# Chatit-cloud/BEE2BEE

Measured on AMD Instinct MI355X. Metric: output tokens/sec (llama3-8b bf16 greedy decode, replica peers), higher is better.
Workload: dtype bf16; 1 GPU; model=llama3-8b, global_batch=1536, seq_len=1024, parallelism=replica-dp1, decode_graphs=True, distinct_prompts=256

## Files before the change

bee2bee_amd/engine/runner.py:

```python
from __future__ import annotations

from typing import List, Optional, Tuple

import torch
import torch.nn.functional as F

from .. import ops
from ..models.spec import ModelSpec
from ..models.weights import ModelWeights
from .kv import PagedKV


class Runner:
    def __init__(
        self,
        spec: ModelSpec,
        weights: ModelWeights,
        kv: PagedKV,
        device: torch.device,
        dtype: torch.dtype = torch.bfloat16,
        layer_range: Optional[Tuple[int, int]] = None,
        window: Optional[int] = None,
    ) -> None:
        self.spec = spec
        self.weights = weights
        self.kv = kv
        self.device = device
        self.dtype = dtype
        self.layer_lo, self.layer_hi = layer_range or (0, spec.n_layers)
        self.scale = spec.head_dim**-0.5
        self.window = int(
            (spec.sliding_window or 0) if window is None else window)
        self.ep = None
        self.tp_group = None
        self.decode_attn_fn = None
        self.kv_observer = None
        cos, sin = ops.rope_tables(
            spec.max_seq_len, spec.head_dim, spec.rope_theta, device,
            scaling=spec.rope_scaling,
        )
        self.rope_cos, self.rope_sin = cos, sin

    @property
    def is_first_stage(self) -> bool:
        return self.layer_lo == 0

    @property
    def is_last_stage(self) -> bool:
        return self.layer_hi == self.spec.n_layers


    def embed(self, input_ids: torch.Tensor,
              positions: Optional[torch.Tensor] = None) -> torch.Tensor:
        h = F.embedding(input_ids, self.weights.embed)
        if self.spec.pos_type == "learned" and positions is not None:
            h = h + F.embedding(positions.long(), self.weights.pos_embed)
        return h

    def _norm(self, x, w, b):
        if self.spec.norm_type == "layernorm":
            return ops.layernorm(x, w, b, self.spec.rms_eps)
        return ops.rmsnorm(x, w, self.spec.rms_eps)

    def _fused_add_norm(self, x, resid, w, b):
        if self.spec.norm_type == "layernorm":
            return ops.fused_add_layernorm(x, resid, w, b, self.spec.rms_eps)
        return ops.fused_add_rmsnorm(x, resid, w, self.spec.rms_eps)

    def lm_head(self, hidden: torch.Tensor) -> torch.Tensor:
        normed = self._norm(hidden, self.weights.final_norm,
                            self.weights.final_norm_bias)
        return F.linear(normed, self.weights.lm_head)

    def _layer(
        self,
        layer_idx: int,
        hidden: torch.Tensor,
        residual: Optional[torch.Tensor],
        positions: torch.Tensor,
        slot_mapping: torch.Tensor,
        attn_fn,
    ) -> Tuple[torch.Tensor, torch.Tensor]:
        s = self.spec
        lw = self.weights.layers[layer_idx]
        if residual is None:
            residual = hidden
            normed = self._norm(hidden, lw.attn_norm, lw.attn_norm_bias)
        else:
            normed, residual = self._fused_add_norm(
                hidden, residual, lw.attn_norm, lw.attn_norm_bias
            )

        qkv = F.linear(normed, lw.wqkv)
        if lw.wqkv_bias is not None:
            qkv = qkv + lw.wqkv_bias
        T = qkv.shape[0]
        q, k, v = qkv.split([s.q_size, s.kv_size, s.kv_size], dim=-1)
        q = q.view(T, s.n_heads, s.head_dim)
        k = k.view(T, s.n_kv_heads, s.head_dim)
        v = v.view(T, s.n_kv_heads, s.head_dim)
        if s.qk_norm:
            ops.qk_norm_rope_inplace(q, k, positions, self.rope_cos,
                                     self.rope_sin, lw.q_norm, lw.k_norm,
                                     s.rms_eps)
        elif s.pos_type == "rope":
            ops.rope_inplace(q, k, positions, self.rope_cos, self.rope_sin)
        if self.kv_observer is not None:
            self.kv_observer(layer_idx, k, v)
        k_cache, v_cache = self.kv.layer(layer_idx)
        sc = self.kv.layer_scales(layer_idx)
        if sc is None:
            ops.kv_cache_store(k, v, k_cache, v_cache, slot_mapping)
        else:
            ops.kv_cache_store(k, v, k_cache, v_cache, slot_mapping,
                               k_inv_scale=sc[2], v_inv_scale=sc[3])
        attn_out = attn_fn(layer_idx, q, k, v, k_cache, v_cache)
        attn_out = F.linear(attn_out.reshape(T, s.q_size), lw.wo, lw.wo_bias)
        if self.tp_group is not None:
            import torch.distributed as dist

            dist.all_reduce(attn_out, group=self.tp_group)

        normed, residual = self._fused_add_norm(
            attn_out, residual, lw.mlp_norm, lw.mlp_norm_bias
        )
        if s.is_moe:
            mlp_out = self._moe_mlp(lw, normed)
        elif s.act_type == "gelu":
            fc = F.linear(normed, lw.w_gate_up, lw.w_gate_up_bias)
            mlp_out = F.linear(ops.gelu(fc), lw.w_down, lw.w_down_bias)
        else:
            gate_up = F.linear(normed, lw.w_gate_up)
            mlp_out = F.linear(ops.swiglu(gate_up), lw.w_down)
            if self.tp_group is not None:
                import torch.distributed as dist

                dist.all_reduce(mlp_out, group=self.tp_group)
        return mlp_out, residual

# ... 83 lines not shown
            out.index_add_(
                0, tok, contrib * weights.reshape(-1).unsqueeze(-1)
            )
            return out.to(x.dtype)

        out = torch.zeros_like(x, dtype=torch.float32)
        for e in range(E):
            mask = idx == e
            if not bool(mask.any()):
                continue
            tok, kslot = mask.nonzero(as_tuple=True)
            xe = x[tok]
            ge = F.linear(xe, lw.moe_w_gate_up[e])
            ye = F.linear(ops.swiglu(ge), lw.moe_w_down[e])
            out.index_add_(0, tok, ye.float() * weights[tok, kslot, None])
        return out.to(x.dtype)

    def _run_layers(
        self,
        hidden: torch.Tensor,
        positions: torch.Tensor,
        slot_mapping: torch.Tensor,
        attn_fn,
    ) -> torch.Tensor:
        residual = None
        for layer_idx in range(self.layer_lo, self.layer_hi):
            hidden, residual = self._layer(
                layer_idx, hidden, residual, positions, slot_mapping, attn_fn
            )
        return hidden + residual if residual is not None else hidden

    def forward_prefill(
        self,
        input_ids_or_hidden: torch.Tensor,
        positions: torch.Tensor,
        slot_mapping: torch.Tensor,
        cu_seqlens: torch.Tensor,
        max_seqlen: int,
        block_table: Optional[torch.Tensor] = None,
        seq_lens: Optional[torch.Tensor] = None,
        query_lens: Optional[torch.Tensor] = None,
    ) -> torch.Tensor:
        chunked = seq_lens is not None

        def attn(layer_idx, q, k, v, k_cache, v_cache):
            if chunked:
                sc = self.kv.layer_scales(layer_idx)
                kw = {} if sc is None else {"k_scale": sc[0],
                                            "v_scale": sc[1]}
                if self.window:
                    kw["window"] = self.window
# ... 25 lines not shown
        def attn(layer_idx, q, k, v, k_cache, v_cache):
            sc = self.kv.layer_scales(layer_idx)
            kw = {} if sc is None else {"k_scale": sc[0], "v_scale": sc[1]}
            if self.decode_attn_fn is not None:
                if self.window:
                    raise ValueError(
                        "sliding-window attention is not supported with an "
                        "injected (context-parallel) decode attention")
                return self.decode_attn_fn(
                    q, k_cache, v_cache, block_table, seq_lens, self.scale,
                    **kw
                )
            if self.window:
                kw["window"] = self.window
            return ops.attn_decode(
                q, k_cache, v_cache, block_table, seq_lens, self.scale, **kw
            )

        hidden = (
            self.embed(input_ids_or_hidden, positions)
            if self.is_first_stage
            else input_ids_or_hidden
        )
        return self._run_layers(hidden, positions, slot_mapping, attn)
```

bee2bee_amd/ops/__init__.py:

```python
from __future__ import annotations

import os
from typing import Optional, Tuple

import torch

from . import reference

_hip = None
_hip_err: Optional[str] = None


def _load_hip():
    global _hip, _hip_err
    if _hip is not None or _hip_err is not None:
        return _hip
    try:
        import importlib

        _hip = importlib.import_module("bee2bee_amd.ops._bee2bee_hip")
    except Exception as e:
        _hip_err = str(e)
        _hip = None
    return _hip
# ... 139 lines not shown
    q: torch.Tensor,
    k_cache: torch.Tensor,
    v_cache: torch.Tensor,
    block_table: torch.Tensor,
    seq_lens: torch.Tensor,
    scale: float,
    k_scale: Optional[torch.Tensor] = None,
    v_scale: Optional[torch.Tensor] = None,
    window: int = 0,
    path="auto",
    max_z: int = 0,
):
    if _use_hip(q):
        out, ml = require_hip().attn_decode_select(
            q, k_cache, v_cache, block_table, seq_lens, scale, k_scale,
            v_scale, window, _DECODE_PATHS.get(path, path), max_z
        )
        return out, ml
    return reference.attn_decode_lse(
        q, k_cache, v_cache, block_table, seq_lens, scale,
        k_scale=k_scale, v_scale=v_scale, window=window)


def attn_prefill(
    q: torch.Tensor,
    k: torch.Tensor,
    v: torch.Tensor,
    cu_seqlens: torch.Tensor,
    max_seqlen: int,
    scale: float,
    causal: bool = True,
    window: int = 0,
) -> torch.Tensor:
    if _use_hip(q):
        return require_hip().attn_prefill(
            q, k, v, cu_seqlens, max_seqlen, scale, causal, window
        )
    return reference.attn_prefill(q, k, v, cu_seqlens, max_seqlen, scale,
                                  causal, window=window)


def attn_prefill_paged(
    q: torch.Tensor,
    k_cache: torch.Tensor,
    v_cache: torch.Tensor,
    block_table: torch.Tensor,
# ... 57 lines not shown
```

bee2bee_amd/ops/csrc/attn_decode.hip:

```cpp
#include "common.h"

#define DEC_BLOCK 256
#define DEC_WAVES 4
#define DEC_CHUNK 256

template <typename KVT>
__device__ __forceinline__ bf16x8 load_kv_bf16x8(const KVT* p);
template <>
__device__ __forceinline__ bf16x8 load_kv_bf16x8(const unsigned short* p) {
    return *reinterpret_cast<const bf16x8*>(p);
}
template <>
__device__ __forceinline__ bf16x8 load_kv_bf16x8(const unsigned char* p) {
    float f[8];
    load_fp8x8(p, f);
    bf16x8 r;
#pragma unroll
    for (int e = 0; e < 8; ++e) r[e] = (__bf16)f[e];
    return r;
}
template <typename KVT> struct kv_pair_t;
template <> struct kv_pair_t<unsigned short> { short2v v; };
template <> struct kv_pair_t<unsigned char> { u8x2 v; };
__device__ __forceinline__ float2v kv_pair_f32(kv_pair_t<unsigned short> p) {
// ... 710 lines not shown
    for (int c = c0; c < nc; ++c) Ltot += __expf(ml_s[c][0] - M) * ml_s[c][1];
    const float inv = (Ltot > 0.f) ? 1.f / Ltot : 0.f;
    if (out_ml != nullptr && threadIdx.x == 0) {
        float* mlrow = out_ml + ((long)b * nq + kvh * G + g) * 2;
        mlrow[0] = M;
        mlrow[1] = Ltot;
    }

    for (int d = threadIdx.x; d < hd; d += DEC_BLOCK) {
        float acc = 0.f;
        for (int c = c0; c < nc; ++c)
            acc += __expf(ml_s[c][0] - M) *
                   part_o[((base + c) * G + g) * hd + d];
        out[((long)b * nq + kvh * G + g) * hd + d] = f2bf(acc * inv);
    }
}

__device__ __forceinline__ int phase_tid() {
    int t = threadIdx.x;
    asm volatile("" : "+v"(t));
    return t;
}

template <int G, int HD, bool FOLD, typename KVT, bool SCALED, bool WINDOWED>
__global__ __launch_bounds__(DEC_BLOCK)
__attribute__((amdgpu_waves_per_eu(4))) void attn_decode_fused_kernel(
    const unsigned short* __restrict__ q,
    const KVT* __restrict__ k_cache,
    const KVT* __restrict__ v_cache,
    const int* __restrict__ block_table,
    const int* __restrict__ seq_lens,
    float* __restrict__ part_o,
    float* __restrict__ part_ml,
    unsigned short* __restrict__ out,
    float* __restrict__ out_ml,
    int nkv, int W, int bs, int C, long q_stride, float scale,
    const float* __restrict__ k_scale,
    const float* __restrict__ v_scale,
    int window) {
    constexpr int KSTEPS = HD / 32;
    constexpr int TILES = WAVE / 16;
    const int b = blockIdx.x;
    const int kvh = blockIdx.y;
    const int nq = nkv * G;
    const int L = seq_lens[b];
    const int lo = WINDOWED ? max(0, L - window) : 0;
    const int c0 = WINDOWED ? lo / DEC_CHUNK : 0;
    if ((c0 + (int)blockIdx.z) * DEC_CHUNK >= L) {
        if (FOLD && L <= 0) {
            unsigned short* orow = out + ((long)b * nq + kvh * G) * HD;
            for (int i = threadIdx.x; i < G * HD; i += DEC_BLOCK) orow[i] = 0;
            if (out_ml != nullptr && threadIdx.x < G) {
                float* mlrow =
                    out_ml + ((long)b * nq + kvh * G + threadIdx.x) * 2;
                mlrow[0] = -1e30f;
                mlrow[1] = 0.f;
            }
        }
        return;
    }
    float ksc = 1.f, vsc = 1.f;
    if (SCALED) {
        ksc = k_scale[kvh];
        vsc = v_scale[kvh];
    }
    extern __shared__ __attribute__((aligned(16))) char smem_raw[];
    float* p_s = reinterpret_cast<float*>(smem_raw);
    long* voff_s = reinterpret_cast<long*>(p_s + DEC_CHUNK * G);
    float* merge = reinterpret_cast<float*>(voff_s + DEC_CHUNK);
    float* run = merge + DEC_WAVES * G * HD;
    unsigned short* q_s = reinterpret_cast<unsigned short*>(run + G * HD);
    float* red = reinterpret_cast<float*>(
        reinterpret_cast<char*>(q_s) + ((G * HD * 2 + 15) & ~15));
    float* runml = red + DEC_WAVES * G * 2;

    {
    const int lane = threadIdx.x % WAVE;
    const int wid = threadIdx.x / WAVE;
    if (SCALED) {
        float amax = 0.f;
        for (int i = threadIdx.x; i < G * HD; i += DEC_BLOCK) {
            const int g = i / HD, d = i % HD;
            amax = fmaxf(amax, fabsf(bf2f(f2bf(
                bf2f(q[(long)b * q_stride + (kvh * G + g) * (long)HD + d]) *
                scale))));
        }
        amax = wave_max(amax);
        if (lane == 0) red[wid] = amax;
        __syncthreads();
        amax = fmaxf(fmaxf(red[0], red[1]), fmaxf(red[2], red[3]));
        const int e = __builtin_amdgcn_readfirstlane(
            (__float_as_int(amax) >> 23) & 0xff);
        float qmul = 1.f;
        if (e >= 8 && e < 122) {
            qmul = __int_as_float((261 - e) << 23);
            ksc *= __int_as_float((e - 7) << 23);
        }
        for (int i = threadIdx.x; i < G * HD; i += DEC_BLOCK) {
            const int g = i / HD, d = i % HD;
            q_s[i] = f2bf(bf2f(f2bf(
                bf2f(q[(long)b * q_stride + (kvh * G + g) * (long)HD + d]) *
                scale)) * qmul);
// ... 258 lines not shown

template <int G, int HD, typename KVT, bool WIN>
static void launch_scores_mfma(
    dim3 grid, int smem, hipStream_t stream, const unsigned short* q,
    const KVT* kc, const int* block_table, const int* seq_lens,
    unsigned short* p_buf, float* part_ml, int nkv, int W, int bs, int C,
    long q_stride, float scale, const float* k_scale, int window) {
    if constexpr (sizeof(KVT) == 1) {
        if (k_scale != nullptr) {
            hipLaunchKernelGGL(
                (attn_scores_mfma_kernel<G, HD, KVT, true, WIN>), grid,
                dim3(DEC_BLOCK), smem, stream, q, kc, block_table, seq_lens,
                p_buf, part_ml, nkv, W, bs, C, q_stride, scale, k_scale,
                window);
            return;
        }
    }
    hipLaunchKernelGGL((attn_scores_mfma_kernel<G, HD, KVT, false, WIN>),
                       grid, dim3(DEC_BLOCK), smem, stream, q, kc,
                       block_table, seq_lens, p_buf, part_ml, nkv, W, bs, C,
                       q_stride, scale, nullptr, window);
}

template <int G, int HD, typename KVT, bool WIN>
static void launch_fused(
    dim3 grid, int smem, hipStream_t stream, const unsigned short* q,
    const KVT* kc, const KVT* vc, const int* block_table,
    const int* seq_lens, float* part_o, float* part_ml, unsigned short* out,
    float* out_ml, int nkv, int W, int bs, int C, long q_stride, float scale,
    const float* k_scale, const float* v_scale, int window) {
#define FUSED_GO(FOLD, SC)                                                     \
    hipLaunchKernelGGL(                                                        \
        (attn_decode_fused_kernel<G, HD, FOLD, KVT, SC, WIN>), grid,           \
        dim3(DEC_BLOCK), smem, stream, q, kc, vc, block_table, seq_lens,       \
        part_o, part_ml, out, out_ml, nkv, W, bs, C, q_stride, scale,          \
        k_scale, v_scale, window)
    const bool fold = grid.z == 1;
    if constexpr (sizeof(KVT) == 1) {
        if (k_scale != nullptr) {
            if (fold) FUSED_GO(true, true);
            else FUSED_GO(false, true);
            return;
        }
    }
    if (fold) FUSED_GO(true, false);
    else FUSED_GO(false, false);
#undef FUSED_GO
}

static bool pv_mfma_enabled() {
    static int pv_mfma = -1;
    if (pv_mfma < 0) {
        const char* e = getenv("BEE2BEE_PV_MFMA");
        pv_mfma = (e != nullptr && e[0] == '1') ? 1 : 0;
    }
    return pv_mfma == 1;
}

#define DEC_FUSED_AUTO_BF16 1
#define DEC_FUSED_AUTO_FP8 1
extern "C" void attn_decode_plan(int B, int nkv, int hd, int C, int fp8,
                                 int path, int max_z, int* Z_out,
                                 int* fused_out) {
    int Z = (4096 + B * nkv - 1) / (B * nkv);
    if (Z > C) Z = C;
    if (max_z > 0 && Z > max_z) Z = max_z;
    if (Z < 1) Z = 1;
    *Z_out = Z;
    const bool can = hd == 64 || hd == 128;
    if (path == 0)
        *fused_out = can && !pv_mfma_enabled() &&
                     (fp8 ? DEC_FUSED_AUTO_FP8 : DEC_FUSED_AUTO_BF16);
    else
        *fused_out = path == 2 && can;
}

extern "C" void launch_attn_decode(
    const unsigned short* q, const void* k_cache, const void* v_cache,
    const int* block_table, const int* seq_lens, unsigned short* p_buf,
    float* part_o, float* part_ml, unsigned short* out, float* out_ml,
    int B, int nkv,
    int G, int W, int bs, int hd, int C, long q_stride, float scale,
    int fp8, const float* k_scale, const float* v_scale, int window,
    int path, int max_z, hipStream_t stream) {
    int Z, fused;
    attn_decode_plan(B, nkv, hd, C, fp8, path, max_z, &Z, &fused);
    const bool pv_mfma = pv_mfma_enabled();
    dim3 grid(B, nkv, Z);
    dim3 cgrid(B, nkv, G);
    const int smem_s = ((G * hd * 2 + 15) & ~15) + DEC_WAVES * G * 2 * 4;
    const int smem_pv = DEC_CHUNK * G * 4 + DEC_CHUNK * 8 +
                        DEC_WAVES * G * hd * 4 +
                        G * hd * 4 + G * 8;
    const int smem_pvm = ((G * (DEC_CHUNK + 8) * 2 + 15) & ~15) +
                         DEC_CHUNK * 8 + 2 * hd * PVM_STRIDE * 2;
    const int smem_f = smem_pv + smem_s;
#define LAUNCH_T(GG, KVT, WIN)                                                 \
    do {                                                                       \
        const KVT* kc = reinterpret_cast<const KVT*>(k_cache);                 \
        const KVT* vc = reinterpret_cast<const KVT*>(v_cache);                 \
        if (fused) {                                                           \
            if (hd == 128)                                                     \
                launch_fused<GG, 128, KVT, WIN>(                               \
                    grid, smem_f, stream, q, kc, vc, block_table, seq_lens,    \
                    part_o, part_ml, out, out_ml, nkv, W, bs, C, q_stride,     \
                    scale, k_scale, v_scale, window);                          \
            else                                                               \
                launch_fused<GG, 64, KVT, WIN>(                                \
                    grid, smem_f, stream, q, kc, vc, block_table, seq_lens,    \
                    part_o, part_ml, out, out_ml, nkv, W, bs, C, q_stride,     \
                    scale, k_scale, v_scale, window);                          \
            if (Z > 1)                                                         \
                hipLaunchKernelGGL((attn_decode_combine_kernel<GG, WIN>),      \
                                   cgrid, dim3(DEC_BLOCK), 0, stream, part_o,  \
                                   part_ml, seq_lens, out, out_ml, nkv, hd, C, \
                                   window);                                    \
            break;                                                             \
        }                                                                      \
        if (hd == 128)                                                         \
            launch_scores_mfma<GG, 128, KVT, WIN>(                             \
                grid, smem_s, stream, q, kc, block_table, seq_lens, p_buf,     \
                part_ml, nkv, W, bs, C, q_stride, scale, k_scale, window);     \
        else if (hd == 64)                                                     \
            launch_scores_mfma<GG, 64, KVT, WIN>(                              \
                grid, smem_s, stream, q, kc, block_table, seq_lens, p_buf,     \
                part_ml, nkv, W, bs, C, q_stride, scale, k_scale, window);     \
        else                                                                   \
            hipLaunchKernelGGL((attn_scores_kernel<GG, KVT, WIN>), grid,       \
                               dim3(DEC_BLOCK), smem_s, stream, q, kc,         \
                               block_table, seq_lens, p_buf, part_ml, nkv, W,  \
                               bs, hd, C, q_stride, scale, k_scale, window);   \
        if (!WIN && hd == 128 && pv_mfma && !fp8) {                            \
            hipLaunchKernelGGL(attn_pv_mfma_kernel<GG>, grid,                  \
                               dim3(DEC_BLOCK), smem_pvm, stream,              \
// ... 24 lines not shown
#define LAUNCH(GG)                                                             \
    do {                                                                       \
        if (window > 0) {                                                      \
            if (fp8) LAUNCH_T(GG, unsigned char, true);                        \
            else LAUNCH_T(GG, unsigned short, true);                           \
        } else {                                                               \
            if (fp8) LAUNCH_T(GG, unsigned char, false);                       \
            else LAUNCH_T(GG, unsigned short, false);                          \
        }                                                                      \
    } while (0)
    switch (G) {
        case 1: LAUNCH(1); break;
        case 2: LAUNCH(2); break;
        case 3: LAUNCH(3); break;
        case 4: LAUNCH(4); break;
        case 5: LAUNCH(5); break;
        case 6: LAUNCH(6); break;
        case 7: LAUNCH(7); break;
        case 8: LAUNCH(8); break;
        default: LAUNCH(16); break;
    }
#undef LAUNCH
#undef LAUNCH_T
}
```

bee2bee_amd/ops/csrc/common.h:

```cpp
#pragma once

#include <hip/hip_runtime.h>
#include <hip/hip_bf16.h>

#define WAVE 64

typedef __attribute__((ext_vector_type(8))) __bf16 bf16x8;
typedef __attribute__((ext_vector_type(4))) float f32x4;
typedef __attribute__((ext_vector_type(8))) short short8;
typedef __attribute__((ext_vector_type(2))) short short2v;
typedef __attribute__((ext_vector_type(2))) float float2v;
typedef __attribute__((ext_vector_type(8))) unsigned char uchar8;
typedef __attribute__((ext_vector_type(2))) unsigned char u8x2;

__device__ __forceinline__ unsigned short f2fp8x2(float a, float b) {
    return (unsigned short)(__builtin_amdgcn_cvt_pk_fp8_f32(a, b, 0, false) &
                            0xffff);
}
__device__ __forceinline__ float2v fp8x2_2f(unsigned short w) {
    return __builtin_amdgcn_cvt_pk_f32_fp8((int)w, false);
}
__device__ __forceinline__ void load_fp8x8(const unsigned char* p,
                                           float* out) {
    const unsigned int* pi = reinterpret_cast<const unsigned int*>(p);
    const unsigned int w0 = pi[0], w1 = pi[1];
    const float2v a = __builtin_amdgcn_cvt_pk_f32_fp8((int)w0, false);
    const float2v b = __builtin_amdgcn_cvt_pk_f32_fp8((int)w0, true);
    const float2v c = __builtin_amdgcn_cvt_pk_f32_fp8((int)w1, false);
    const float2v d = __builtin_amdgcn_cvt_pk_f32_fp8((int)w1, true);
    out[0] = a.x; out[1] = a.y; out[2] = b.x; out[3] = b.y;
    out[4] = c.x; out[5] = c.y; out[6] = d.x; out[7] = d.y;
}

__device__ __forceinline__ float bf2f(unsigned short u) {
    union { unsigned int i; float f; } v;
    v.i = ((unsigned int)u) << 16;
    return v.f;
}

__device__ __forceinline__ unsigned short f2bf(float f) {
    union { unsigned int i; float f; } v;
    v.f = f;
    unsigned int rounding = 0x7FFF + ((v.i >> 16) & 1);
// ... 52 lines not shown
```

bee2bee_amd/ops/csrc/elementwise.hip:

```cpp
#include "common.h"

template <bool FUSED_ADD>
__global__ void rmsnorm_kernel(
    const unsigned short* __restrict__ x,
    const unsigned short* __restrict__ resid,
    const unsigned short* __restrict__ w,
    unsigned short* __restrict__ y,
    unsigned short* __restrict__ resid_out,
    int H, float eps) {
    extern __shared__ __attribute__((aligned(16))) char smem_raw[];
    float* row = reinterpret_cast<float*>(smem_raw);
    __shared__ float red[8];

    const long t = blockIdx.x;
    const unsigned short* xr = x + t * (long)H;
    const unsigned short* rr = FUSED_ADD ? resid + t * (long)H : nullptr;
    unsigned short* ro = FUSED_ADD ? resid_out + t * (long)H : nullptr;

    float sumsq = 0.f;
    for (int i = threadIdx.x * 8; i < H; i += blockDim.x * 8) {
        float v[8];
        load_bf16x8(xr + i, v);
        if (FUSED_ADD) {
            float r[8];
// ... 207 lines not shown
    unsigned short* __restrict__ k_cache,
    unsigned short* __restrict__ v_cache,
    const int* __restrict__ slots,
    int T, int nkv, int hd, int bs, long sk, long sv) {
    const int glob_wave = (blockIdx.x * blockDim.x + threadIdx.x) / WAVE;
    const int lane = threadIdx.x % WAVE;
    if (glob_wave >= T * nkv) return;
    const int t = glob_wave / nkv;
    const int h = glob_wave % nkv;
    const int slot = slots[t];
    const int blk = slot / bs, off = slot % bs;
    const long dst = (((long)blk * nkv + h) * bs + off) * hd;
    const unsigned short* ks = k + (long)t * sk + (long)h * hd;
    const unsigned short* vs = v + (long)t * sv + (long)h * hd;
    for (int d = lane * 2; d + 1 < hd; d += WAVE * 2) {
        *reinterpret_cast<short2v*>(k_cache + dst + d) =
            *reinterpret_cast<const short2v*>(ks + d);
        *reinterpret_cast<short2v*>(v_cache + dst + d) =
            *reinterpret_cast<const short2v*>(vs + d);
    }
    if (hd % 2) {  }
}

__device__ __forceinline__ float clamp_e4m3(float x) {
    return fminf(fmaxf(x, -448.f), 448.f);
}

__global__ void kv_store_fp8_kernel(
    const unsigned short* __restrict__ k,
    const unsigned short* __restrict__ v,
    unsigned char* __restrict__ k_cache,
    unsigned char* __restrict__ v_cache,
    const int* __restrict__ slots,
    const float* __restrict__ k_inv,
    const float* __restrict__ v_inv,
    int T, int nkv, int hd, int bs, long sk, long sv) {
    const int glob_wave = (blockIdx.x * blockDim.x + threadIdx.x) / WAVE;
    const int lane = threadIdx.x % WAVE;
    if (glob_wave >= T * nkv) return;
    const int t = glob_wave / nkv;
    const int h = glob_wave % nkv;
    const int slot = slots[t];
    const int blk = slot / bs, off = slot % bs;
    const long dst = (((long)blk * nkv + h) * bs + off) * hd;
    const unsigned short* ks = k + (long)t * sk + (long)h * hd;
    const unsigned short* vs = v + (long)t * sv + (long)h * hd;
    if (k_inv != nullptr) {
        const int hu = __builtin_amdgcn_readfirstlane(h);
        const float ki = k_inv[hu], vi = v_inv[hu];
// ... 147 lines not shown
```

bee2bee_amd/ops/csrc/ext.cpp:

```cpp
#include <torch/extension.h>
#include <ATen/hip/HIPContext.h>
#include <hip/hip_runtime.h>

#include <climits>

using torch::Tensor;

extern "C" {
void launch_rmsnorm(const unsigned short*, const unsigned short*,
                    unsigned short*, long, int, float, hipStream_t);
void launch_fused_add_rmsnorm(const unsigned short*, const unsigned short*,
                              const unsigned short*, unsigned short*,
                              unsigned short*, long, int, float, hipStream_t);
void launch_layernorm(const unsigned short*, const unsigned short*,
                      const unsigned short*, unsigned short*, long, int,
                      float, hipStream_t);
void launch_fused_add_layernorm(const unsigned short*, const unsigned short*,
                                const unsigned short*, const unsigned short*,
                                unsigned short*, unsigned short*, long, int,
                                float, hipStream_t);
void launch_gelu(const unsigned short*, unsigned short*, long, hipStream_t);
void launch_rope(unsigned short*, unsigned short*, const int*, const float*,
                 const float*, int, int, int, int, long, long, hipStream_t);
void launch_qk_norm_rope(unsigned short*, unsigned short*, const int*,
                         const float*, const float*, const unsigned short*,
                         const unsigned short*, int, int, int, int, long,
                         long, float, hipStream_t);
void launch_kv_store(const unsigned short*, const unsigned short*,
                     unsigned short*, unsigned short*, const int*, int, int,
                     int, int, long, long, hipStream_t);
void launch_kv_store_fp8(const unsigned short*, const unsigned short*,
                         unsigned char*, unsigned char*, const int*,
                         const float*, const float*, int, int, int, int, long,
                         long, hipStream_t);
void launch_swiglu(const unsigned short*, unsigned short*, long, long,
                   hipStream_t);
void launch_attn_decode(const unsigned short*, const void*, const void*,
                        const int*, const int*, unsigned short*, float*,
                        float*, unsigned short*, float*, int, int, int, int,
                        int, int, int, long, float, int, const float*,
                        const float*, int, int, int, hipStream_t);
void attn_decode_plan(int, int, int, int, int, int, int, int*, int*);
void launch_attn_prefill(const unsigned short*, const unsigned short*,
                         const unsigned short*, const int*, unsigned short*,
                         int, int, int, int, long, long, long, int, float,
                         int, int, hipStream_t);
void launch_attn_prefill_paged(const unsigned short*, const void*,
                               const void*, const int*, const int*,
                               const int*, unsigned short*, int, int, int,
                               int, long, int, int, int, float, int,
                               const float*, const float*, int, hipStream_t);
void launch_mfma_probe(const unsigned short*, const unsigned short*, float*,
                       hipStream_t);
void launch_mfma_probe_fp8(const unsigned char*, const unsigned char*,
                           float*, hipStream_t);
void launch_grouped_gemm(const unsigned short*, const unsigned short*,
                         const int*, unsigned short*, int, int, int, int,
                         hipStream_t);
void launch_bw_linear(const unsigned short*, long, float*, hipStream_t);
void launch_bw_rowperlane(const unsigned short*, long, int, int, float*,
                          hipStream_t);
void launch_bw_rowperinstr(const unsigned short*, long, int, int, float*,
                           hipStream_t);
void launch_bw_paged(const unsigned short*, const int*, long, int, int,
                     float*, hipStream_t);
// ... 293 lines not shown
                                    const Tensor& v_cache,
                                    const Tensor& block_table,
                                    const Tensor& seq_lens, double scale,
                                    const OptTensor& k_scale,
                                    const OptTensor& v_scale,
                                    int64_t window) {
    return attn_decode_impl(q, k_cache, v_cache, block_table, seq_lens,
                            scale, k_scale, v_scale, window, true);
}

std::vector<Tensor> attn_decode_select(const Tensor& q, const Tensor& k_cache,
                                       const Tensor& v_cache,
                                       const Tensor& block_table,
                                       const Tensor& seq_lens, double scale,
                                       const OptTensor& k_scale,
                                       const OptTensor& v_scale,
                                       int64_t window, int64_t path,
                                       int64_t max_z) {
    return attn_decode_impl(q, k_cache, v_cache, block_table, seq_lens,
                            scale, k_scale, v_scale, window, true, path,
                            max_z);
}

Tensor attn_prefill(const Tensor& q, const Tensor& k, const Tensor& v,
                    const Tensor& cu_seqlens, long max_seqlen, double scale,
                    bool causal, int64_t window) {
    check_bf16(q, "q");
    check_bf16(k, "k");
    TORCH_CHECK(window >= 0 && window <= INT_MAX,
                "attn_prefill: window must be >= 0 (0 = off)");
    TORCH_CHECK(window == 0 || causal,
                "attn_prefill: a sliding window needs causal attention");
    TORCH_CHECK(cu_seqlens.scalar_type() == torch::kInt32 &&
                cu_seqlens.is_contiguous());
    const int T = q.size(0), nq = q.size(1), hd = q.size(2);
    const int nkv = k.size(1);
    const int nseq = cu_seqlens.size(0) - 1;
    TORCH_CHECK(nq % nkv == 0);
    TORCH_CHECK(q.stride(2) == 1 && q.stride(1) == hd);
    TORCH_CHECK(k.stride(2) == 1 && k.stride(1) == hd);
    TORCH_CHECK(v.stride(2) == 1 && v.stride(1) == hd);
    Tensor out = torch::empty({T, nq, hd}, q.options());
    launch_attn_prefill(bf16p(q), bf16p(k), bf16p(v),
                        cu_seqlens.data_ptr<int>(), bf16p_mut(out), nseq, nq,
                        nkv, hd, q.stride(0), k.stride(0), v.stride(0),
                        (int)max_seqlen, (float)scale, causal ? 1 : 0,
// ... 122 lines not shown
          py::arg("v_inv_scale") = py::none());
    m.def("swiglu", &swiglu, "silu(g) * u");
    m.def("layernorm", &layernorm, "LayerNorm (bf16, weight+bias)");
    m.def("fused_add_layernorm", &fused_add_layernorm,
          "residual add + LayerNorm");
    m.def("gelu", &gelu, "gelu_new (tanh approximation)");
    m.def("attn_decode", &attn_decode, "paged GQA decode attention",
          py::arg("q"), py::arg("k_cache"), py::arg("v_cache"),
          py::arg("block_table"), py::arg("seq_lens"), py::arg("scale"),
          py::arg("k_scale") = py::none(), py::arg("v_scale") = py::none(),
          py::arg("window") = 0);
    m.def("attn_decode_lse", &attn_decode_lse,
          "paged GQA decode attention + per-head (m, l) merge state",
          py::arg("q"), py::arg("k_cache"), py::arg("v_cache"),
          py::arg("block_table"), py::arg("seq_lens"), py::arg("scale"),
          py::arg("k_scale") = py::none(), py::arg("v_scale") = py::none(),
          py::arg("window") = 0);
    m.def("attn_decode_select", &attn_decode_select,
          "attn_decode_lse with an explicit kernel path and Z cap",
          py::arg("q"), py::arg("k_cache"), py::arg("v_cache"),
          py::arg("block_table"), py::arg("seq_lens"), py::arg("scale"),
          py::arg("k_scale") = py::none(), py::arg("v_scale") = py::none(),
          py::arg("window") = 0, py::arg("path") = 0, py::arg("max_z") = 0);
    m.def("attn_prefill", &attn_prefill, "varlen causal flash prefill",
          py::arg("q"), py::arg("k"), py::arg("v"), py::arg("cu_seqlens"),
          py::arg("max_seqlen"), py::arg("scale"), py::arg("causal"),
          py::arg("window") = 0);
    m.def("attn_prefill_paged", &attn_prefill_paged,
          "chunked prefill vs paged history", py::arg("q"),
          py::arg("k_cache"), py::arg("v_cache"), py::arg("block_table"),
          py::arg("seq_lens"), py::arg("cu_q"), py::arg("max_qlen"),
          py::arg("scale"), py::arg("k_scale") = py::none(),
          py::arg("v_scale") = py::none(), py::arg("window") = 0);
    m.def("mfma_probe", &mfma_probe, "16x16x32 bf16 MFMA layout probe");
    m.def("mfma_probe_fp8", &mfma_probe_fp8,
          "16x16x32 fp8 MFMA layout probe");
    m.def("grouped_gemm", &grouped_gemm, "per-expert segment GEMM (MoE)");
    m.def("bw_probe", &bw_probe, "bandwidth pattern probe");
    m.def("bw_probe_paged", &bw_probe_paged, "paged row-per-lane probe");
}
```

Before: 27770 tokens/s.

## Fuse RoPE and KV-cache append into the fused decode attention kernel

Result: no change. 27930 tokens/s, median of 6 (+0.6%).

```diff
diff --git a/bee2bee_amd/engine/runner.py b/bee2bee_amd/engine/runner.py
--- a/bee2bee_amd/engine/runner.py
+++ b/bee2bee_amd/engine/runner.py
@@ -35,6 +35,7 @@
         self.tp_group = None
         self.decode_attn_fn = None
         self.kv_observer = None
+        self.fuse_decode_prologue = True
         cos, sin = ops.rope_tables(
             spec.max_seq_len, spec.head_dim, spec.rope_theta, device,
             scaling=spec.rope_scaling,
@@ -80,6 +81,7 @@
         positions: torch.Tensor,
         slot_mapping: torch.Tensor,
         attn_fn,
+        decode_ctx=None,
     ) -> Tuple[torch.Tensor, torch.Tensor]:
         s = self.spec
         lw = self.weights.layers[layer_idx]
@@ -99,22 +101,35 @@
         q = q.view(T, s.n_heads, s.head_dim)
         k = k.view(T, s.n_kv_heads, s.head_dim)
         v = v.view(T, s.n_kv_heads, s.head_dim)
-        if s.qk_norm:
-            ops.qk_norm_rope_inplace(q, k, positions, self.rope_cos,
-                                     self.rope_sin, lw.q_norm, lw.k_norm,
-                                     s.rms_eps)
-        elif s.pos_type == "rope":
-            ops.rope_inplace(q, k, positions, self.rope_cos, self.rope_sin)
-        if self.kv_observer is not None:
-            self.kv_observer(layer_idx, k, v)
         k_cache, v_cache = self.kv.layer(layer_idx)
         sc = self.kv.layer_scales(layer_idx)
-        if sc is None:
-            ops.kv_cache_store(k, v, k_cache, v_cache, slot_mapping)
+        if decode_ctx is not None and ops.attn_decode_rope_store_fuses(
+                q, k_cache, decode_ctx[0], self.window):
+            kw = {} if sc is None else {
+                "k_scale": sc[0], "v_scale": sc[1],
+                "k_inv_scale": sc[2], "v_inv_scale": sc[3]}
+            if self.window:
+                kw["window"] = self.window
+            attn_out = ops.attn_decode_rope_store(
+                q, k, v, positions, self.rope_cos, self.rope_sin, k_cache,
+                v_cache, slot_mapping, decode_ctx[0], decode_ctx[1],
+                self.scale, **kw)
         else:
-            ops.kv_cache_store(k, v, k_cache, v_cache, slot_mapping,
-                               k_inv_scale=sc[2], v_inv_scale=sc[3])
-        attn_out = attn_fn(layer_idx, q, k, v, k_cache, v_cache)
+            if s.qk_norm:
+                ops.qk_norm_rope_inplace(q, k, positions, self.rope_cos,
+                                         self.rope_sin, lw.q_norm, lw.k_norm,
+                                         s.rms_eps)
+            elif s.pos_type == "rope":
+                ops.rope_inplace(q, k, positions, self.rope_cos,
+                                 self.rope_sin)
+            if self.kv_observer is not None:
+                self.kv_observer(layer_idx, k, v)
+            if sc is None:
+                ops.kv_cache_store(k, v, k_cache, v_cache, slot_mapping)
+            else:
+                ops.kv_cache_store(k, v, k_cache, v_cache, slot_mapping,
+                                   k_inv_scale=sc[2], v_inv_scale=sc[3])
+            attn_out = attn_fn(layer_idx, q, k, v, k_cache, v_cache)
         attn_out = F.linear(attn_out.reshape(T, s.q_size), lw.wo, lw.wo_bias)
         if self.tp_group is not None:
             import torch.distributed as dist
@@ -244,11 +259,13 @@
         positions: torch.Tensor,
         slot_mapping: torch.Tensor,
         attn_fn,
+        decode_ctx=None,
     ) -> torch.Tensor:
         residual = None
         for layer_idx in range(self.layer_lo, self.layer_hi):
             hidden, residual = self._layer(
-                layer_idx, hidden, residual, positions, slot_mapping, attn_fn
+                layer_idx, hidden, residual, positions, slot_mapping, attn_fn,
+                decode_ctx
             )
         return hidden + residual if residual is not None else hidden
 
@@ -320,4 +337,8 @@
             if self.is_first_stage
             else input_ids_or_hidden
         )
-        return self._run_layers(hidden, positions, slot_mapping, attn)
+        fuse = (self.fuse_decode_prologue and self.spec.pos_type == "rope"
+                and not self.spec.qk_norm and self.kv_observer is None
+                and self.decode_attn_fn is None)
+        return self._run_layers(hidden, positions, slot_mapping, attn,
+                                (block_table, seq_lens) if fuse else None)
diff --git a/bee2bee_amd/ops/__init__.py b/bee2bee_amd/ops/__init__.py
--- a/bee2bee_amd/ops/__init__.py
+++ b/bee2bee_amd/ops/__init__.py
@@ -185,6 +185,86 @@
         k_scale=k_scale, v_scale=v_scale, window=window)
 
 
+def attn_decode_rope_store_lse(
+    q: torch.Tensor,
+    k: torch.Tensor,
+    v: torch.Tensor,
+    positions: torch.Tensor,
+    cos: torch.Tensor,
+    sin: torch.Tensor,
+    k_cache: torch.Tensor,
+    v_cache: torch.Tensor,
+    slot_mapping: torch.Tensor,
+    block_table: torch.Tensor,
+    seq_lens: torch.Tensor,
+    scale: float,
+    k_scale: Optional[torch.Tensor] = None,
+    v_scale: Optional[torch.Tensor] = None,
+    k_inv_scale: Optional[torch.Tensor] = None,
+    v_inv_scale: Optional[torch.Tensor] = None,
+    window: int = 0,
+    path="auto",
+    max_z: int = 0,
+):
+    if _use_hip(q):
+        out, ml = require_hip().attn_decode_rope_store(
+            q, k, v, positions, cos, sin, k_cache, v_cache, slot_mapping,
+            block_table, seq_lens, scale, k_scale, v_scale, k_inv_scale,
+            v_inv_scale, window, True, _DECODE_PATHS.get(path, path), max_z
+        )
+        return out, ml
+    q2, k2 = q.clone(), k.clone()
+    reference.rope_inplace(q2, k2, positions, cos, sin)
+    reference.kv_cache_store(k2, v, k_cache, v_cache, slot_mapping,
+                             k_inv_scale, v_inv_scale)
+    return reference.attn_decode_lse(
+        q2, k_cache, v_cache, block_table, seq_lens, scale,
+        k_scale=k_scale, v_scale=v_scale, window=window)
+
+
+def attn_decode_rope_store_fuses(q: torch.Tensor, k_cache: torch.Tensor,
+                                 block_table: torch.Tensor,
+                                 window: int = 0) -> bool:
+    if _use_hip(q):
+        return require_hip().attn_decode_rope_store_fuses(
+            q, k_cache, block_table, window)
+    return True
+
+
+def attn_decode_rope_store(
+    q: torch.Tensor,
+    k: torch.Tensor,
+    v: torch.Tensor,
+    positions: torch.Tensor,
+    cos: torch.Tensor,
+    sin: torch.Tensor,
+    k_cache: torch.Tensor,
+    v_cache: torch.Tensor,
+    slot_mapping: torch.Tensor,
+    block_table: torch.Tensor,
+    seq_lens: torch.Tensor,
+    scale: float,
+    k_scale: Optional[torch.Tensor] = None,
+    v_scale: Optional[torch.Tensor] = None,
+    k_inv_scale: Optional[torch.Tensor] = None,
+    v_inv_scale: Optional[torch.Tensor] = None,
+    window: int = 0,
+) -> torch.Tensor:
+    if _use_hip(q):
+        return require_hip().attn_decode_rope_store(
+            q, k, v, positions, cos, sin, k_cache, v_cache, slot_mapping,
+            block_table, seq_lens, scale, k_scale, v_scale, k_inv_scale,
+            v_inv_scale, window
+        )[0]
+    q2, k2 = q.clone(), k.clone()
+    reference.rope_inplace(q2, k2, positions, cos, sin)
+    reference.kv_cache_store(k2, v, k_cache, v_cache, slot_mapping,
+                             k_inv_scale, v_inv_scale)
+    return reference.attn_decode(q2, k_cache, v_cache, block_table, seq_lens,
+                                 scale, k_scale=k_scale, v_scale=v_scale,
+                                 window=window)
+
+
 def attn_prefill(
     q: torch.Tensor,
     k: torch.Tensor,
diff --git a/bee2bee_amd/ops/csrc/attn_decode.hip b/bee2bee_amd/ops/csrc/attn_decode.hip
--- a/bee2bee_amd/ops/csrc/attn_decode.hip
+++ b/bee2bee_amd/ops/csrc/attn_decode.hip
@@ -756,12 +756,55 @@
     return t;
 }
 
-template <int G, int HD, bool FOLD, typename KVT, bool SCALED, bool WINDOWED>
+struct DecPrologue {
+    const unsigned short* k_new;
+    const unsigned short* v_new;
+    long k_stride, v_stride;
+    const int* positions;
+    const float* cos_t;
+    const float* sin_t;
+    const int* slots;
+    const float* k_inv;
+    const float* v_inv;
+};
+template <typename KVT, bool PRO> struct dec_cache_ptr {
+    using type = const KVT* __restrict__;
+};
+template <typename KVT> struct dec_cache_ptr<KVT, true> {
+    using type = KVT*;
+};
+
+__device__ __forceinline__ void rope_pair(float x1, float x2, float c,
+                                          float s, unsigned short* r1,
+                                          unsigned short* r2) {
+#pragma clang fp contract(off)
+    const float x2s = x2 * s;
+    const float x2c = x2 * c;
+    *r1 = f2bf(__builtin_fmaf(x1, c, -x2s));
+    *r2 = f2bf(__builtin_fmaf(x1, s, x2c));
+}
+
+template <bool SC>
+__device__ __forceinline__ unsigned short cache_elem(unsigned short*,
+                                                     unsigned short x,
+                                                     float) {
+    return x;
+}
+template <bool SC>
+__device__ __forceinline__ unsigned char cache_elem(unsigned char*,
+                                                    unsigned short x,
+                                                    float inv) {
+    const float f = SC ? clamp_e4m3(bf2f(x) * inv) : bf2f(x);
+    return (unsigned char)(f2fp8x2(f, f) & 0xff);
+}
+
+template <int G, int HD, bool FOLD, typename KVT, bool SCALED, bool WINDOWED,
+          bool PRO>
 __global__ __launch_bounds__(DEC_BLOCK)
 __attribute__((amdgpu_waves_per_eu(4))) void attn_decode_fused_kernel(
     const unsigned short* __restrict__ q,
-    const KVT* __restrict__ k_cache,
-    const KVT* __restrict__ v_cache,
+    typename dec_cache_ptr<KVT, PRO>::type k_cache,
+    typename dec_cache_ptr<KVT, PRO>::type v_cache,
     const int* __restrict__ block_table,
     const int* __restrict__ seq_lens,
     float* __restrict__ part_o,
@@ -771,7 +814,8 @@
     int nkv, int W, int bs, int C, long q_stride, float scale,
     const float* __restrict__ k_scale,
     const float* __restrict__ v_scale,
-    int window) {
+    int window,
+    DecPrologue pro) {
     constexpr int KSTEPS = HD / 32;
     constexpr int TILES = WAVE / 16;
     const int b = blockIdx.x;
@@ -811,7 +855,74 @@
     {
     const int lane = threadIdx.x % WAVE;
     const int wid = threadIdx.x / WAVE;
-    if (SCALED) {
+    if constexpr (PRO) {
+        constexpr int HALF = HD / 2;
+        const long tab = (long)pro.positions[b] * HALF;
+        for (int p = threadIdx.x; p < G * HALF; p += DEC_BLOCK) {
+            const int g = p / HALF, d = p % HALF;
+            const unsigned short* qh =
+                q + (long)b * q_stride + (kvh * G + g) * (long)HD;
+            unsigned short r1, r2;
+            rope_pair(bf2f(qh[d]), bf2f(qh[d + HALF]), pro.cos_t[tab + d],
+                      pro.sin_t[tab + d], &r1, &r2);
+            q_s[g * HD + d] = SCALED ? r1 : f2bf(bf2f(r1) * scale);
+            q_s[g * HD + d + HALF] = SCALED ? r2 : f2bf(bf2f(r2) * scale);
+        }
+        if (((L - 1) / DEC_CHUNK - c0) % (int)gridDim.z == (int)blockIdx.z) {
+            const int slot = pro.slots[b];
+            BB_KASSERT(slot == block_table[(long)b * W + (L - 1) / bs] * bs +
+                                   (L - 1) % bs);
+            const long dst =
+                (((long)(slot / bs) * nkv + kvh) * bs + slot % bs) * HD;
+            float kinv = 1.f, vinv = 1.f;
+            if (SCALED) {
+                kinv = pro.k_inv[kvh];
+                vinv = pro.v_inv[kvh];
+            }
+            if (wid == 0 && lane < HALF) {
+                const unsigned short* kn =
+                    pro.k_new + (long)b * pro.k_stride + (long)kvh * HD;
+                unsigned short r1, r2;
+                rope_pair(bf2f(kn[lane]), bf2f(kn[lane + HALF]),
+                          pro.cos_t[tab + lane], pro.sin_t[tab + lane], &r1,
+                          &r2);
+                KVT* kd = k_cache + dst;
+                kd[lane] = cache_elem<SCALED>(kd, r1, kinv);
+                kd[lane + HALF] = cache_elem<SCALED>(kd, r2, kinv);
+            } else if (wid == 1 && lane < HALF) {
+                const unsigned short* vn =
+                    pro.v_new + (long)b * pro.v_stride + (long)kvh * HD;
+                const short2v vv =
+                    *reinterpret_cast<const short2v*>(vn + lane * 2);
+                KVT* vd = v_cache + dst;
+                vd[lane * 2] =
+                    cache_elem<SCALED>(vd, (unsigned short)vv[0], vinv);
+                vd[lane * 2 + 1] =
+                    cache_elem<SCALED>(vd, (unsigned short)vv[1], vinv);
+            }
+            asm volatile("s_waitcnt vmcnt(0)" ::: "memory");
+        }
+        if (SCALED) {
+            __syncthreads();
+            float amax = 0.f;
+            for (int i = threadIdx.x; i < G * HD; i += DEC_BLOCK)
+                amax = fmaxf(amax,
+                             fabsf(bf2f(f2bf(bf2f(q_s[i]) * scale))));
+            amax = wave_max(amax);
+            if (lane == 0) red[wid] = amax;
+            __syncthreads();
+            amax = fmaxf(fmaxf(red[0], red[1]), fmaxf(red[2], red[3]));
+            const int e = __builtin_amdgcn_readfirstlane(
+                (__float_as_int(amax) >> 23) & 0xff);
+            float qmul = 1.f;
+            if (e >= 8 && e < 122) {
+                qmul = __int_as_float((261 - e) << 23);
+                ksc *= __int_as_float((e - 7) << 23);
+            }
+            for (int i = threadIdx.x; i < G * HD; i += DEC_BLOCK)
+                q_s[i] = f2bf(bf2f(f2bf(bf2f(q_s[i]) * scale)) * qmul);
+        }
+    } else if (SCALED) {
         float amax = 0.f;
         for (int i = threadIdx.x; i < G * HD; i += DEC_BLOCK) {
             const int g = i / HD, d = i % HD;
@@ -1116,19 +1227,38 @@
                        q_stride, scale, nullptr, window);
 }
 
-template <int G, int HD, typename KVT, bool WIN>
+constexpr bool dec_pro_built(int G, int hd, bool fp8, bool windowed) {
+    if (fp8) return true;
+    if (G == 1) return windowed ? hd != 64 : hd != 128;
+    if (G == 4 || G == 16) return !(windowed && hd == 128);
+    return true;
+}
+#define DEC_PRO_FP8_MAX_BLOCKS 1024
+extern "C" int attn_decode_prologue_built(int B, int nkv, int G, int hd,
+                                          int fp8, int window) {
+    if (fp8 && (long)B * nkv > DEC_PRO_FP8_MAX_BLOCKS) return 0;
+    return (hd == 64 || hd == 128) &&
+           dec_pro_built(G, hd, fp8 != 0, window > 0);
+}
+
+template <int G, int HD, typename KVT, bool WIN, bool PRO>
 static void launch_fused(
     dim3 grid, int smem, hipStream_t stream, const unsigned short* q,
-    const KVT* kc, const KVT* vc, const int* block_table,
+    const KVT* kc_in, const KVT* vc_in, const int* block_table,
     const int* seq_lens, float* part_o, float* part_ml, unsigned short* out,
     float* out_ml, int nkv, int W, int bs, int C, long q_stride, float scale,
-    const float* k_scale, const float* v_scale, int window) {
+    const float* k_scale, const float* v_scale, int window,
+    const DecPrologue& pro) {
+    if constexpr (!PRO || dec_pro_built(G, HD, sizeof(KVT) == 1, WIN)) {
+    using cache_t = typename dec_cache_ptr<KVT, PRO>::type;
+    cache_t kc = (cache_t)kc_in;
+    cache_t vc = (cache_t)vc_in;
 #define FUSED_GO(FOLD, SC)                                                     \
     hipLaunchKernelGGL(                                                        \
-        (attn_decode_fused_kernel<G, HD, FOLD, KVT, SC, WIN>), grid,           \
+        (attn_decode_fused_kernel<G, HD, FOLD, KVT, SC, WIN, PRO>), grid,      \
         dim3(DEC_BLOCK), smem, stream, q, kc, vc, block_table, seq_lens,       \
         part_o, part_ml, out, out_ml, nkv, W, bs, C, q_stride, scale,          \
-        k_scale, v_scale, window)
+        k_scale, v_scale, window, pro)
     const bool fold = grid.z == 1;
     if constexpr (sizeof(KVT) == 1) {
         if (k_scale != nullptr) {
@@ -1140,6 +1270,7 @@
     if (fold) FUSED_GO(true, false);
     else FUSED_GO(false, false);
 #undef FUSED_GO
+    }
 }
 
 static bool pv_mfma_enabled() {
@@ -1169,16 +1300,19 @@
         *fused_out = path == 2 && can;
 }
 
-extern "C" void launch_attn_decode(
+static void launch_attn_decode_impl(
     const unsigned short* q, const void* k_cache, const void* v_cache,
     const int* block_table, const int* seq_lens, unsigned short* p_buf,
     float* part_o, float* part_ml, unsigned short* out, float* out_ml,
     int B, int nkv,
     int G, int W, int bs, int hd, int C, long q_stride, float scale,
     int fp8, const float* k_scale, const float* v_scale, int window,
-    int path, int max_z, hipStream_t stream) {
+    int path, int max_z, const DecPrologue* pro, hipStream_t stream) {
     int Z, fused;
     attn_decode_plan(B, nkv, hd, C, fp8, path, max_z, &Z, &fused);
+    if (pro != nullptr &&
+        !(fused && attn_decode_prologue_built(B, nkv, G, hd, fp8, window)))
+        return;
     const bool pv_mfma = pv_mfma_enabled();
     dim3 grid(B, nkv, Z);
     dim3 cgrid(B, nkv, G);
@@ -1189,21 +1323,26 @@
     const int smem_pvm = ((G * (DEC_CHUNK + 8) * 2 + 15) & ~15) +
                          DEC_CHUNK * 8 + 2 * hd * PVM_STRIDE * 2;
     const int smem_f = smem_pv + smem_s;
+#define FUSED_T(GG, KVT, WIN, PRO, PARGS)                                      \
+    do {                                                                       \
+        if (hd == 128)                                                         \
+            launch_fused<GG, 128, KVT, WIN, PRO>(                              \
+                grid, smem_f, stream, q, kc, vc, block_table, seq_lens,        \
+                part_o, part_ml, out, out_ml, nkv, W, bs, C, q_stride, scale,  \
+                k_scale, v_scale, window, PARGS);                              \
+        else                                                                   \
+            launch_fused<GG, 64, KVT, WIN, PRO>(                               \
+                grid, smem_f, stream, q, kc, vc, block_table, seq_lens,        \
+                part_o, part_ml, out, out_ml, nkv, W, bs, C, q_stride, scale,  \
+                k_scale, v_scale, window, PARGS);                              \
+    } while (0)
 #define LAUNCH_T(GG, KVT, WIN)                                                 \
     do {                                                                       \
         const KVT* kc = reinterpret_cast<const KVT*>(k_cache);                 \
         const KVT* vc = reinterpret_cast<const KVT*>(v_cache);                 \
         if (fused) {                                                           \
-            if (hd == 128)                                                     \
-                launch_fused<GG, 128, KVT, WIN>(                               \
-                    grid, smem_f, stream, q, kc, vc, block_table, seq_lens,    \
-                    part_o, part_ml, out, out_ml, nkv, W, bs, C, q_stride,     \
-                    scale, k_scale, v_scale, window);                          \
-            else                                                               \
-                launch_fused<GG, 64, KVT, WIN>(                                \
-                    grid, smem_f, stream, q, kc, vc, block_table, seq_lens,    \
-                    part_o, part_ml, out, out_ml, nkv, W, bs, C, q_stride,     \
-                    scale, k_scale, v_scale, window);                          \
+            if (pro != nullptr) FUSED_T(GG, KVT, WIN, true, *pro);             \
+            else FUSED_T(GG, KVT, WIN, false, DecPrologue{});                  \
             if (Z > 1)                                                         \
                 hipLaunchKernelGGL((attn_decode_combine_kernel<GG, WIN>),      \
                                    cgrid, dim3(DEC_BLOCK), 0, stream, part_o,  \
@@ -1274,4 +1413,37 @@
     }
 #undef LAUNCH
 #undef LAUNCH_T
-}
+#undef FUSED_T
+}
+
+extern "C" void launch_attn_decode(
+    const unsigned short* q, const void* k_cache, const void* v_cache,
+    const int* block_table, const int* seq_lens, unsigned short* p_buf,
+    float* part_o, float* part_ml, unsigned short* out, float* out_ml,
+    int B, int nkv,
+    int G, int W, int bs, int hd, int C, long q_stride, float scale,
+    int fp8, const float* k_scale, const float* v_scale, int window,
+    int path, int max_z, hipStream_t stream) {
+    launch_attn_decode_impl(q, k_cache, v_cache, block_table, seq_lens,
+                            p_buf, part_o, part_ml, out, out_ml, B, nkv, G, W,
+                            bs, hd, C, q_stride, scale, fp8, k_scale, v_scale,
+                            window, path, max_z, nullptr, stream);
+}
+
+extern "C" void launch_attn_decode_rope_store(
+    const unsigned short* q, const unsigned short* k_new,
+    const unsigned short* v_new, long k_stride, long v_stride,
+    const int* positions, const float* cos_t, const float* sin_t,
+    const int* slots, const float* k_inv, const float* v_inv, void* k_cache,
+    void* v_cache, const int* block_table, const int* seq_lens,
+    float* part_o, float* part_ml, unsigned short* out, float* out_ml,
+    int B, int nkv, int G, int W, int bs, int hd, int C, long q_stride,
+    float scale, int fp8, const float* k_scale, const float* v_scale,
+    int window, int path, int max_z, hipStream_t stream) {
+    const DecPrologue pro{k_new, v_new, k_stride, v_stride, positions,
+                          cos_t, sin_t, slots, k_inv, v_inv};
+    launch_attn_decode_impl(q, k_cache, v_cache, block_table, seq_lens,
+                            nullptr, part_o, part_ml, out, out_ml, B, nkv, G,
+                            W, bs, hd, C, q_stride, scale, fp8, k_scale,
+                            v_scale, window, path, max_z, &pro, stream);
+}
diff --git a/bee2bee_amd/ops/csrc/common.h b/bee2bee_amd/ops/csrc/common.h
--- a/bee2bee_amd/ops/csrc/common.h
+++ b/bee2bee_amd/ops/csrc/common.h
@@ -19,6 +19,9 @@
 }
 __device__ __forceinline__ float2v fp8x2_2f(unsigned short w) {
     return __builtin_amdgcn_cvt_pk_f32_fp8((int)w, false);
+}
+__device__ __forceinline__ float clamp_e4m3(float x) {
+    return fminf(fmaxf(x, -448.f), 448.f);
 }
 __device__ __forceinline__ void load_fp8x8(const unsigned char* p,
                                            float* out) {
diff --git a/bee2bee_amd/ops/csrc/elementwise.hip b/bee2bee_amd/ops/csrc/elementwise.hip
--- a/bee2bee_amd/ops/csrc/elementwise.hip
+++ b/bee2bee_amd/ops/csrc/elementwise.hip
@@ -253,9 +253,6 @@
     if (hd % 2) {  }
 }
 
-__device__ __forceinline__ float clamp_e4m3(float x) {
-    return fminf(fmaxf(x, -448.f), 448.f);
-}
 
 __global__ void kv_store_fp8_kernel(
     const unsigned short* __restrict__ k,
diff --git a/bee2bee_amd/ops/csrc/ext.cpp b/bee2bee_amd/ops/csrc/ext.cpp
--- a/bee2bee_amd/ops/csrc/ext.cpp
+++ b/bee2bee_amd/ops/csrc/ext.cpp
@@ -40,7 +40,14 @@
                         float*, unsigned short*, float*, int, int, int, int,
                         int, int, int, long, float, int, const float*,
                         const float*, int, int, int, hipStream_t);
+void launch_attn_decode_rope_store(
+    const unsigned short*, const unsigned short*, const unsigned short*, long,
+    long, const int*, const float*, const float*, const int*, const float*,
+    const float*, void*, void*, const int*, const int*, float*, float*,
+    unsigned short*, float*, int, int, int, int, int, int, int, long, float,
+    int, const float*, const float*, int, int, int, hipStream_t);
 void attn_decode_plan(int, int, int, int, int, int, int, int*, int*);
+int attn_decode_prologue_built(int, int, int, int, int, int);
 void launch_attn_prefill(const unsigned short*, const unsigned short*,
                          const unsigned short*, const int*, unsigned short*,
                          int, int, int, int, long, long, long, int, float,
@@ -380,6 +387,131 @@
                             max_z);
 }
 
+std::vector<Tensor> attn_decode_rope_store(
+    const Tensor& q, const Tensor& k, const Tensor& v, const Tensor& pos,
+    const Tensor& cos_t, const Tensor& sin_t, Tensor& k_cache,
+    Tensor& v_cache, const Tensor& slots, const Tensor& block_table,
+    const Tensor& seq_lens, double scale, const OptTensor& k_scale,
+    const OptTensor& v_scale, const OptTensor& k_inv_scale,
+    const OptTensor& v_inv_scale, int64_t window, bool want_lse,
+    int64_t path, int64_t max_z) {
+    check_bf16(q, "q");
+    check_bf16(k, "k");
+    check_bf16(v, "v");
+    TORCH_CHECK(path >= 0 && path <= 2,
+                "attn_decode: path is 0 (auto), 1 (split) or 2 (fused)");
+    TORCH_CHECK(max_z >= 0 && max_z <= INT_MAX,
+                "attn_decode: max_z must be >= 0 (0 = no cap)");
+    TORCH_CHECK(window >= 0 && window <= INT_MAX,
+                "attn_decode: window must be >= 0 (0 = off)");
+    const bool scaled =
+        check_kv_scales(k_scale, v_scale, k_cache, "attn_decode_rope_store");
+    const bool inv_scaled = check_kv_scales(k_inv_scale, v_inv_scale, k_cache,
+                                            "attn_decode_rope_store");
+    TORCH_CHECK(scaled == inv_scaled,
+                "attn_decode_rope_store: give the scales and their "
+                "reciprocals together or neither");
+    const bool fp8 = k_cache.scalar_type() == torch::kUInt8;
+    if (!fp8) check_bf16(k_cache, "k_cache");
+    TORCH_CHECK(v_cache.scalar_type() == k_cache.scalar_type() &&
+                v_cache.sizes() == k_cache.sizes());
+    TORCH_CHECK(q.dim() == 3 && k.dim() == 3 && v.dim() == 3 &&
+                k_cache.dim() == 4);
+    const int B = q.size(0), nq = q.size(1), hd = q.size(2);
+    const int nkv = k_cache.size(1), bs = k_cache.size(2);
+    const int W = block_table.size(1);
+    TORCH_CHECK(nq % nkv == 0);
+    const int G = nq / nkv;
+    const int kDecChunk = 256;
+    const int C = (W * bs + kDecChunk - 1) / kDecChunk;
+    TORCH_CHECK(path != 2 || hd == 64 || hd == 128,
+                "attn_decode: the fused kernel supports head_dim 64 and 128, "
+                "got ", hd);
+    int Z = 1, fused = 0;
+    attn_decode_plan(B, nkv, hd, C, fp8 ? 1 : 0, (int)path, (int)max_z, &Z,
+                     &fused);
+    if (!fused ||
+        !attn_decode_prologue_built(B, nkv, G, hd, fp8 ? 1 : 0,
+                                    (int)window)) {
+        Tensor q2 = q.clone(), k2 = k.clone();
+        rope_inplace(q2, k2, pos, cos_t, sin_t);
+        kv_cache_store(k2, v, k_cache, v_cache, slots, k_inv_scale,
+                       v_inv_scale);
+        return attn_decode_impl(q2, k_cache, v_cache, block_table, seq_lens,
+                                scale, k_scale, v_scale, window, want_lse,
+                                path, max_z);
+    }
+    for (const Tensor* t : {&pos, &slots, &block_table, &seq_lens})
+        TORCH_CHECK(t->is_cuda() && t->scalar_type() == torch::kInt32 &&
+                        t->is_contiguous(),
+                    "attn_decode_rope_store: positions, slot_mapping, "
+                    "block_table and seq_lens must be int32 contiguous on "
+                    "GPU");
+    TORCH_CHECK(pos.dim() == 1 && pos.size(0) == B && slots.dim() == 1 &&
+                slots.size(0) == B && seq_lens.size(0) == B &&
+                block_table.dim() == 2 && block_table.size(0) == B);
+    TORCH_CHECK(cos_t.is_cuda() && sin_t.is_cuda() &&
+                cos_t.scalar_type() == torch::kFloat32 &&
+                sin_t.scalar_type() == torch::kFloat32 && cos_t.dim() == 2 &&
+                cos_t.size(1) == hd / 2 && cos_t.sizes() == sin_t.sizes() &&
+                cos_t.is_contiguous() && sin_t.is_contiguous(),
+                "attn_decode_rope_store: cos/sin must be fp32 "
+                "[max_len, head_dim/2] contiguous on GPU");
+    TORCH_CHECK(k.size(0) == B && v.size(0) == B && k.size(1) == nkv &&
+                v.size(1) == nkv && k.size(2) == hd && v.size(2) == hd &&
+                k_cache.size(3) == hd);
+    TORCH_CHECK(G >= 1 && G <= 8 || G == 16,
+                "unsupported GQA group size ", G);
+    TORCH_CHECK(q.stride(2) == 1 && q.stride(1) == hd);
+    TORCH_CHECK(k.stride(2) == 1 && k.stride(1) == hd);
+    TORCH_CHECK(v.stride(2) == 1 && v.stride(1) == hd);
+    TORCH_CHECK(v.stride(0) % 2 == 0 &&
+                reinterpret_cast<uintptr_t>(v.data_ptr()) % 4 == 0);
+    TORCH_CHECK(k_cache.is_contiguous() && v_cache.is_contiguous());
+    TORCH_CHECK(C <= 128, "decode supports up to 32768-token contexts for now");
+    auto fopt = q.options().dtype(torch::kFloat32);
+    Tensor out = torch::empty({B, nq, hd}, q.options());
+    Tensor out_ml, part_o, part_ml;
+    if (want_lse) out_ml = torch::empty({B, nq, 2}, fopt);
+    if (Z > 1) {
+        part_o = torch::empty({B, nkv, C, G, hd}, fopt);
+        part_ml = torch::empty({B, nkv, C, G, 2}, fopt);
+    }
+    if (B > 0)
+    launch_attn_decode_rope_store(
+        bf16p(q), bf16p(k), bf16p(v), k.stride(0), v.stride(0),
+        pos.data_ptr<int>(), cos_t.data_ptr<float>(), sin_t.data_ptr<float>(),
+        slots.data_ptr<int>(),
+        scaled ? k_inv_scale->data_ptr<float>() : nullptr,
+        scaled ? v_inv_scale->data_ptr<float>() : nullptr, k_cache.data_ptr(),
+        v_cache.data_ptr(), block_table.data_ptr<int>(),
+        seq_lens.data_ptr<int>(),
+        part_o.defined() ? part_o.data_ptr<float>() : nullptr,
+        part_ml.defined() ? part_ml.data_ptr<float>() : nullptr,
+        bf16p_mut(out), want_lse ? out_ml.data_ptr<float>() : nullptr, B, nkv,
+        G, W, bs, hd, C, q.stride(0), (float)scale, fp8 ? 1 : 0,
+        scaled ? k_scale->data_ptr<float>() : nullptr,
+        scaled ? v_scale->data_ptr<float>() : nullptr, (int)window, (int)path,
+        (int)max_z, stream());
+    if (want_lse) return {out, out_ml};
+    return {out};
+}
+
+bool attn_decode_rope_store_fuses(const Tensor& q, const Tensor& k_cache,
+                                  const Tensor& block_table,
+                                  int64_t window) {
+    const int B = q.size(0), nq = q.size(1), hd = q.size(2);
+    const int nkv = k_cache.size(1), bs = k_cache.size(2);
+    const int W = block_table.size(1);
+    const bool fp8 = k_cache.scalar_type() == torch::kUInt8;
+    if (nkv == 0 || nq % nkv != 0 || B == 0) return false;
+    const int C = (W * bs + 255) / 256;
+    int Z = 1, fused = 0;
+    attn_decode_plan(B, nkv, hd, C, fp8 ? 1 : 0, 0, 0, &Z, &fused);
+    return fused && attn_decode_prologue_built(B, nkv, nq / nkv, hd,
+                                               fp8 ? 1 : 0, (int)window);
+}
+
 Tensor attn_prefill(const Tensor& q, const Tensor& k, const Tensor& v,
                     const Tensor& cu_seqlens, long max_seqlen, double scale,
                     bool causal, int64_t window) {
@@ -548,6 +680,21 @@
           py::arg("block_table"), py::arg("seq_lens"), py::arg("scale"),
           py::arg("k_scale") = py::none(), py::arg("v_scale") = py::none(),
           py::arg("window") = 0, py::arg("path") = 0, py::arg("max_z") = 0);
+    m.def("attn_decode_rope_store", &attn_decode_rope_store,
+          "RoPE + KV append + paged GQA decode attention in one launch",
+          py::arg("q"), py::arg("k"), py::arg("v"), py::arg("positions"),
+          py::arg("cos"), py::arg("sin"), py::arg("k_cache"),
+          py::arg("v_cache"), py::arg("slot_mapping"), py::arg("block_table"),
+          py::arg("seq_lens"), py::arg("scale"),
+          py::arg("k_scale") = py::none(), py::arg("v_scale") = py::none(),
+          py::arg("k_inv_scale") = py::none(),
+          py::arg("v_inv_scale") = py::none(), py::arg("window") = 0,
+          py::arg("want_lse") = false, py::arg("path") = 0,
+          py::arg("max_z") = 0);
+    m.def("attn_decode_rope_store_fuses", &attn_decode_rope_store_fuses,
+          "does attn_decode_rope_store run as one launch for these shapes",
+          py::arg("q"), py::arg("k_cache"), py::arg("block_table"),
+          py::arg("window") = 0);
     m.def("attn_prefill", &attn_prefill, "varlen causal flash prefill",
           py::arg("q"), py::arg("k"), py::arg("v"), py::arg("cu_seqlens"),
           py::arg("max_seqlen"), py::arg("scale"), py::arg("causal"),
```
